# spaceandtimefdn/blitzar

Hardware: NVIDIA H100
Metric: MSM throughput (scalar*point terms/sec), ristretto255, n=2^20 per GPU (higher is better)
Workload: dtype u32 limbs (integer modular arithmetic)

## Files before the change

### blitzar_b200/build.py

```python
import os
import subprocess
import sys

ROOT = os.path.dirname(os.path.dirname(os.path.abspath(__file__)))
CSRC = os.path.join(ROOT, "blitzar_b200", "csrc")
LIBDIR = os.path.join(ROOT, "blitzar_b200", "lib")
LIB = os.path.join(LIBDIR, "libblitzar_b200.so")
NVCC = os.environ.get("NVCC", "/usr/local/cuda/bin/nvcc")
ARCH = ["-gencode", "arch=compute_90a,code=sm_90a"]
NVCC_FLAGS = ["-std=c++17", "-O3"] + ARCH + ["-lineinfo",
              "--expt-relaxed-constexpr", "-Xcompiler", "-fPIC"]
UNITS = ["api.cu", "curve_ed25519.cu", "curve_bls12381.cu", "curve_bn254.cu", "curve_grumpkin.cu"]


def _newer(target, sources):
    if not os.path.exists(target):
        return True
    t = os.path.getmtime(target)
    return any(os.path.getmtime(s) > t for s in sources)


def _headers():
    return [os.path.join(CSRC, f) for f in os.listdir(CSRC) if f.endswith((".cuh", ".h"))] + \
        [os.path.join(ROOT, "include", "blitzar_b200.h")]
# ... 1 lines not shown

def build_product(verbose=False):
    os.makedirs(LIBDIR, exist_ok=True)
    subprocess.check_call([sys.executable, os.path.join(CSRC, "gen_constants.py")])
    units = [u for u in UNITS if os.path.exists(os.path.join(CSRC, u))]
    objs, procs = [], []
    for u in units:
        src = os.path.join(CSRC, u)
        obj = os.path.join(LIBDIR, u.replace(".cu", ".o"))
        objs.append(obj)
        if _newer(obj, [src, os.path.abspath(__file__)] + _headers()):
            cmd = [NVCC] + NVCC_FLAGS + (["-Xptxas", "-v"] if verbose else []) + ["-c", src, "-o", obj]
            procs.append((u, subprocess.Popen(cmd, stdout=subprocess.PIPE, stderr=subprocess.STDOUT)))
    for u, p in procs:
        out, _ = p.communicate()
        if verbose or p.returncode:
            sys.stderr.write(out.decode())
        if p.returncode:
            raise RuntimeError(f"nvcc failed for {u}")
    if procs or not os.path.exists(LIB):
        subprocess.check_call([NVCC, "-shared"] + ARCH + ["-o", LIB] + objs +
                              ["-Xlinker", "--version-script=" + os.path.join(CSRC, "export.map")])
    return LIB


def build_emul():
    edir = os.path.join(ROOT, "tests", "emul")
    out = os.path.join(edir, "libb200_emul.so")
    objdir = os.path.join(edir, "obj")
    os.makedirs(objdir, exist_ok=True)
    prefix = os.path.join(edir, "emul_prefix.h")
    flags = ["g++", "-std=c++17", "-O1", "-DB200_EMULATE", "-fPIC", "-w", "-include", prefix]
    jobs, objs = [], []
    harness = ["emul.cpp", "ptable_emul.cpp", "offsets_emul.cpp", "partition_msm_emul.cpp"]
    for u in [x for x in UNITS if x.startswith("curve_")] + harness:
        src = os.path.join(edir if u in harness else CSRC, u)
        obj = os.path.join(objdir, u.rsplit(".", 1)[0] + ".o")
        objs.append(obj)
        if _newer(obj, [src, prefix] + _headers()):
            jobs.append((u, subprocess.Popen(flags + ["-x", "c++", "-c", src, "-o", obj],
                                             stdout=subprocess.PIPE, stderr=subprocess.STDOUT)))
    for u, p in jobs:
        o, _ = p.communicate()
        if p.returncode:
            sys.stderr.write(o.decode())
            raise RuntimeError(f"emulation build failed for {u}")
    if jobs or not os.path.exists(out):
        subprocess.check_call(["g++", "-shared", "-o", out] + objs)
    return out


def build_oracle_port():
    src = os.path.join(ROOT, "oracle", "msm_oracle.c")
    out = os.path.join(ROOT, "oracle", "libmsm_oracle.so")
    if os.path.exists(src) and _newer(out, [src]):
        subprocess.check_call(["gcc", "-O2", "-fPIC", "-shared", "-w", src, "-o", out])
    return out


def build_oracle_ref():
    ref = os.environ.get("BLITZAR_REFERENCE")
    if not ref or not os.path.isdir(os.path.join(ref, "sxt")):
        return None
    subprocess.check_call(["make", "-s", "-j8", "-C", os.path.join(ROOT, "oracle", "ref_build"),
                           "R=" + os.path.abspath(ref)], stdout=subprocess.DEVNULL)
    return os.path.join(ROOT, "oracle", "_ref", "libblitzar_ref_cpu.so")

# ... 11 lines not shown
```

### blitzar_b200/csrc/api.cu

```cuda
#include <algorithm>
#include <cctype>
#include <cstdint>
#include <cstdio>
#include <cstdlib>
#include <cstring>
#include <condition_variable>
#include <functional>
#include <mutex>
#include <thread>
#include <memory>
#include <string>
#include <vector>

#include "engine_api.cuh"

using namespace b200;

namespace {

struct State {
  bool initialized = false;
  int device = -1;
  cudaStream_t stream = nullptr;
  cudaStream_t copy_stream = nullptr;
  cudaStream_t tail_stream = nullptr;
  cudaEvent_t range_events[16] = {};
  cudaEvent_t alloc_event = nullptr;
  void* builtin = nullptr;
  uint64_t num_builtin = 0;
  unsigned builtin_window_bits = 0, builtin_windows = 0;
  MsmOptions opt;
};
State g_state;
EngineCtx ctx_of(const State& st) {
  EngineCtx c{st.stream, g_state.opt, st.builtin, st.num_builtin};
  c.builtin_window_bits = st.builtin_window_bits;
  c.builtin_windows = st.builtin_windows;
  static const bool tail_on = [] {
    const char* env = std::getenv("BLITZAR_B200_TAIL_STREAM");
    return env != nullptr && std::atoi(env) != 0;
  }();
  if (tail_on)
    c.tail = st.tail_stream;
  if (const char* env = std::getenv("BLITZAR_B200_GROUP_ENTRIES"))
    c.opt.max_group_entries = std::strtoull(env, nullptr, 10);
  if (const char* env = std::getenv("BLITZAR_B200_UNIFORM_ADD"))
    c.opt.uniform_add = (u32)std::atoi(env);
  if (const char* env = std::getenv("BLITZAR_B200_LANE_TAIL"))
    c.opt.lane_tail = (u32)std::atoi(env);
  if (const char* env = std::getenv("BLITZAR_B200_SCATTER_WM"))
    c.opt.scatter_window_major = (u32)std::atoi(env);
  if (const char* env = std::getenv("BLITZAR_B200_SORT"))
    c.opt.sort_path = (u32)std::atoi(env);
  if (const char* env = std::getenv("BLITZAR_B200_PAIR_LEVELS"))
    c.opt.pair_levels = std::atoi(env);
  if (const char* env = std::getenv("BLITZAR_B200_PAIR_BATCH"))
    c.opt.pair_batch = (u32)std::atoi(env);
  if (const char* env = std::getenv("BLITZAR_B200_TABLE_POLICY"))
    c.opt.table_policy = (u32)std::atoi(env);
  if (const char* env = std::getenv("BLITZAR_B200_PARTITION_POLICY"))
    c.partition_policy = (u32)std::atoi(env);
  return c;
}
EngineCtx ctx() { return ctx_of(g_state); }
std::mutex g_mutex;

void init_device_state(State& st) {
  B200_CUDA(cudaSetDevice(st.device));
  B200_CUDA(cudaStreamCreateWithFlags(&st.stream, cudaStreamNonBlocking));
  B200_CUDA(cudaStreamCreateWithFlags(&st.copy_stream, cudaStreamNonBlocking));
  int prio_low = 0, prio_high = 0;
  B200_CUDA(cudaDeviceGetStreamPriorityRange(&prio_low, &prio_high));
  B200_CUDA(cudaStreamCreateWithPriority(&st.tail_stream, cudaStreamNonBlocking, prio_high));
  for (auto& e : st.range_events)
    B200_CUDA(cudaEventCreateWithFlags(&e, cudaEventDisableTiming));
  B200_CUDA(cudaEventCreateWithFlags(&st.alloc_event, cudaEventDisableTiming));
  cudaMemPool_t pool;
  B200_CUDA(cudaDeviceGetDefaultMemPool(&pool, st.device));
  uint64_t threshold = UINT64_MAX;
  B200_CUDA(cudaMemPoolSetAttribute(pool, cudaMemPoolAttrReleaseThreshold, &threshold));
}

void ensure_device() {
  if (g_state.stream)
    return;
  int count = 0;
// ... 1318 lines not shown
```

### blitzar_b200/csrc/curve.cuh

```cuda
#pragma once
#include "field.cuh"

namespace b200 {

enum CurveId : unsigned { kRistretto255 = 0, kBls12381 = 1, kBn254 = 2, kGrumpkin = 3 };

struct SeqExec {
  static constexpr int kLanes = 1;
  template <class F>
  static B200_HD void mul4(typename F::E& o0, typename F::E& o1, typename F::E& o2,
                           typename F::E& o3, const typename F::E& a0, const typename F::E& b0,
                           const typename F::E& a1, const typename F::E& b1,
                           const typename F::E& a2, const typename F::E& b2,
                           const typename F::E& a3, const typename F::E& b3) {
    F::mul(o0, a0, b0);
    F::mul(o1, a1, b1);
    F::mul(o2, a2, b2);
    F::mul(o3, a3, b3);
  }
  template <class F>
  static B200_HD void mul2(typename F::E& o0, typename F::E& o1, const typename F::E& a0,
                           const typename F::E& b0, const typename F::E& a1,
                           const typename F::E& b1) {
    F::mul(o0, a0, b0);
// ... 148 lines not shown
    F::select(qt, g.T2d, nt, negate);
    F::sub(t0, a.Y, a.X);
    F::add(t1, a.Y, a.X);
    if (unit_z) {
      F::mul(A, t0, qm);
      F::mul(B, t1, qp);
      F::mul(C, a.T, qt);
      F::dbl(D, a.Z);
    } else {
      X::template mul4<F>(A, B, C, D, t0, qm, t1, qp, a.T, qt, a.Z, g.Z2);
    }
    F::sub(E, B, A);
    F::sub(Fv, D, C);
    F::add(G, D, C);
    F::add(H, B, A);
    Point o;
    X::template mul4<F>(o.X, o.Y, o.T, o.Z, E, Fv, G, H, E, H, Fv, G);
    r = o;
  }
  template <class X = SeqExec> static B200_HD void dbl(Point& r, const Point& a) {
    fe A, B, C, E, Fv, G, H, t0, t1;
    F::add(t0, a.X, a.Y);
    X::template mul4<F>(A, B, C, t1, a.X, a.X, a.Y, a.Y, a.Z, a.Z, t0, t0);
    F::dbl(C, C);
    F::add(H, A, B);
    F::sub(E, H, t1);
    F::sub(G, A, B);
    F::add(Fv, C, G);
    Point o;
    X::template mul4<F>(o.X, o.Y, o.T, o.Z, E, Fv, G, H, E, H, Fv, G);
    r = o;
  }

  static B200_HD void load_gen_abi(Gen& g, const void* src) {
    const u64* s = (const u64*)src;
    Point p;
    F::from_radix51(p.X, s);
    F::from_radix51(p.Y, s + 5);
    F::from_radix51(p.Z, s + 10);
    F::from_radix51(p.T, s + 15);
    point_to_gen(g, p);
  }
  static B200_HD void load_proj_abi(Gen& g, const void* src) { load_gen_abi(g, src); }
  static constexpr int kAbiCompactBytes = 120;
  static B200_HD void load_compact_abi(Gen& g, const void* src) {
    const u64* s = (const u64*)src;
    Point p;
    F::from_radix51(p.X, s);
    F::from_radix51(p.Y, s + 5);
    p.Z = F::one();
    F::from_radix51(p.T, s + 10);
    point_to_gen(g, p);
  }
  static B200_HD void store_compact_abi(void* dst, const Point& p, const fe& zi) {
    u64* d = (u64*)dst;
    fe x, y, t;
    F::mul(x, p.X, zi);
    F::mul(y, p.Y, zi);
    F::mul(t, x, y);
    F::to_radix51(d, x);
    F::to_radix51(d + 5, y);
    F::to_radix51(d + 10, t);
  }
  static B200_HD void store_proj_abi(void* dst, const Point& p) {
    u64* d = (u64*)dst;
    F::to_radix51(d, p.X);
    F::to_radix51(d + 5, p.Y);
    F::to_radix51(d + 10, p.Z);
    F::to_radix51(d + 15, p.T);
  }

  struct ScalarPow {
    static B200_HD void pow22523(fe& r, const fe& a) { F::pow22523(r, a); }
// ... 464 lines not shown
```

### blitzar_b200/csrc/engine.cuh

```cuda
#pragma once
#include <cstdint>
#include <vector>

#include "engine_api.cuh"
#include "msm.cuh"
#include "partition_msm.cuh"
#include "ptable.cuh"
#include "synth.cuh"

namespace b200 {

inline uint64_t check_descriptors(const sxt_sequence_descriptor* d, uint32_t num) {
  B200_REQUIRE(d != nullptr, "descriptors == nullptr");
  uint64_t longest = 0;
  for (uint32_t i = 0; i < num; ++i) {
    B200_REQUIRE(d[i].n == 0 || d[i].data != nullptr, "descriptor.n > 0 with data == nullptr");
    B200_REQUIRE(d[i].element_nbytes != 0 && d[i].element_nbytes <= 32,
                 "descriptor.element_nbytes must be in 1..32");
    if (d[i].is_signed)
      B200_REQUIRE(d[i].element_nbytes <= 16 &&
                       (d[i].element_nbytes & (d[i].element_nbytes - 1)) == 0,
                   "signed columns need a power-of-two element_nbytes <= 16");
    B200_REQUIRE(d[i].n < (1ull << 31), "column too long");
    longest = longest < d[i].n ? d[i].n : longest;
// ... 9 lines not shown
                          Point* out, u32 num_ranges = 1, RangeHook* hook = nullptr) {
    const uint64_t kMaxEntries = ctx.opt.max_group_entries;
    size_t b = 0;
    while (b < cols.size()) {
      size_t e = b;
      uint64_t entries = 0;
      while (e < cols.size()) {
        uint64_t est = (uint64_t)cols[e].n * (cols[e].bit_width / 10 + 1);
        if (e > b && entries + est > kMaxEntries)
          break;
        entries += est;
        ++e;
      }
      std::vector<ColumnDesc> group(cols.begin() + b, cols.begin() + e);
      const bool whole = b == 0 && e == cols.size();
      if (!whole && hook && b == 0) {
        hook->before_range(0, ~0ull);
        hook->before_accumulate();
      }
      msm_run<C>(ctx.s, gens, group, out + b, ctx.opt, whole ? num_ranges : 1,
                 whole ? hook : nullptr, ctx.tail);
      b = e;
    }
  }

  struct IngestHook : RangeHook {
    const EngineCtx* ctx;
    const unsigned char* raw;
    Gen* gens;
    uint64_t n, offset_generators;
    bool builtin;
    range_wait_fn wait;
    void* wait_user;
    bool pending = false;
    void before_range(u64 begin, u64 end) override {
      if (end > n)
        end = n;
      if (begin >= end)
        return;
      if (wait)
        wait(wait_user, begin, end);
      if (raw) {
        stream_t aux = aux_stream();
        stream_follow(aux, ctx->s);
        launch(IngestBody<C, false>{raw + begin * C::kAbiGenBytes, gens + begin}, end - begin, aux);
        pending = true;
      } else if (builtin) {
        launch_builtin(ctx->s, gens + begin, offset_generators + begin, end - begin);
      }
    }
    void before_accumulate() override {
      if (pending) {
        stream_follow(ctx->s, aux_stream());
        pending = false;
      }
    }
  };
  static void launch_builtin(stream_t s, Gen* gens, uint64_t first, uint64_t count) {
    if constexpr (C::kCurveId == kRistretto255)
      launch(BuiltinGeneratorBody{gens, first}, count, s);
    else
      die("generators == nullptr", __FILE__, __LINE__);
  }

  struct PiecesHook : RangeHook {
    const EngineCtx* ctx;
    const GenLayout* layout;
    const unsigned char* raw;
    bool packed;
    bool generate;
    Gen* gens;
    range_wait_fn wait;
    void* wait_user;
    bool pending = false;
    void before_range(u64 begin, u64 end) override {
      end = std::min<u64>(end, layout->max_n);
      if (begin >= end)
        return;
      if (wait)
        wait(wait_user, begin, end);
      if (!raw && !generate)
        return;
      const std::vector<GenLayout::Piece> pieces = layout->needed(begin, end);
      const size_t np = pieces.size();
      std::vector<u64> block(3 * np + 1, 0);
      for (size_t k = 0; k < np; ++k) {
        block[k + 1] = block[k] + pieces[k].count;
        block[np + 1 + k] = raw && packed ? pieces[k].pos : pieces[k].src;
        block[2 * np + 1 + k] = pieces[k].pos;
      }
      const stream_t on = raw ? aux_stream() : ctx->s;
      if (raw)
        stream_follow(on, ctx->s);
      const u64* staged = (const u64*)stage_to_device(on, block.data(), block.size() * sizeof(u64));
      const GenPieces p{staged, staged + np + 1, staged + 2 * np + 1, (u32)np};
      if (raw) {
        launch(IngestPiecesBody<C>{raw, gens, p}, block[np], on);
        pending = true;
      } else if constexpr (C::kCurveId == kRistretto255) {
        launch(BuiltinPiecesBody{gens, p}, block[np], on);
      }
      dev_free((void*)staged, on);
    }
    void before_accumulate() override {
      if (pending) {
        stream_follow(ctx->s, aux_stream());
        pending = false;
      }
    }
  };

  static std::vector<ColumnDesc> columns_of(const sxt_sequence_descriptor* d, uint32_t num) {
    std::vector<ColumnDesc> cols(num);
    for (uint32_t i = 0; i < num; ++i) {
      cols[i].base = d[i].data;
      cols[i].row_stride = d[i].element_nbytes;
      cols[i].bit_offset = 0;
      cols[i].bit_width = 8u * d[i].element_nbytes;
      cols[i].n = (u32)d[i].n;
      cols[i].is_signed = d[i].is_signed ? 1u : 0u;
      cols[i].first_window = cols[i].num_windows = 0;
      cols[i].table_n = 0;
    }
    return cols;
  }

  static void commit_columns(const EngineCtx& ctx, void* out_commitments, void* out_partials,
                             std::vector<ColumnDesc>& cols, const Gen* gens, bool builtin_table,
                             uint32_t num_ranges, RangeHook* hook) {
    stream_t s = ctx.s;
// ... 13 lines not shown
    }
    run_columns(rctx, gens, cols, pts, num_ranges ? num_ranges : 1, hook);
    hook->before_accumulate();
    if (out_commitments)
      launch_store_commit<C>(s, pts, (unsigned char*)out_commitments, num, ctx.opt.lane_tail != 0);
  }

  static void commit_device(const EngineCtx& ctx, void* out_commitments, void* out_partials,
                            uint32_t num, const sxt_sequence_descriptor* d,
                            const void* generators_dev, uint64_t offset_generators,
                            uint32_t num_ranges, range_wait_fn wait, void* wait_user) {
    stream_t s = ctx.s;
    uint64_t n = check_descriptors(d, num);
    DevBuf<Gen> gens(n ? n : 1, s);
    const Gen* gens_ptr = gens.p;
    IngestHook hook;
    hook.ctx = &ctx;
    hook.raw = (const unsigned char*)generators_dev;
    hook.gens = gens.p;
    hook.n = n;
    hook.offset_generators = offset_generators;
    hook.builtin = false;
    hook.wait = wait;
    hook.wait_user = wait_user;
    if (n && !generators_dev) {
      if (C::kCurveId != kRistretto255)
        die("generators == nullptr", __FILE__, __LINE__);
      if (offset_generators + n <= ctx.num_builtin)
        gens_ptr = (const Gen*)ctx.builtin + offset_generators;
      else
        hook.builtin = true;
    }
    std::vector<ColumnDesc> cols = columns_of(d, num);
    commit_columns(ctx, out_commitments, out_partials, cols, gens_ptr,
                   n && !generators_dev && !hook.builtin, num_ranges, &hook);
  }

  static void commit_device_offsets(const EngineCtx& ctx, void* out_commitments,
                                    void* out_partials, uint32_t num,
                                    const sxt_sequence_descriptor* d, const void* generators_dev,
                                    const uint64_t* offsets, bool packed, uint32_t num_ranges,
                                    range_wait_fn wait, void* wait_user) {
    check_descriptors(d, num);
    const GenLayout layout(d, num, offsets);
    if (layout.total && !generators_dev && C::kCurveId != kRistretto255)
      die("generators == nullptr", __FILE__, __LINE__);
    const bool builtin_table = layout.total && !generators_dev && layout.within(ctx.num_builtin);
    DevBuf<Gen> gens(builtin_table ? 1 : layout.total, ctx.s);
    PiecesHook hook;
    hook.ctx = &ctx;
    hook.layout = &layout;
    hook.raw = (const unsigned char*)generators_dev;
    hook.packed = packed;
    hook.generate = layout.total && !generators_dev && !builtin_table;
    hook.gens = gens.p;
    hook.wait = wait;
    hook.wait_user = wait_user;
    std::vector<ColumnDesc> cols = columns_of(d, num);
    for (uint32_t j = 0; j < num; ++j)
      cols[j].gen_base = builtin_table && d[j].n && offsets ? (u32)offsets[j] : layout.base[j];
    commit_columns(ctx, out_commitments, out_partials, cols,
                   builtin_table ? (const Gen*)ctx.builtin : gens.p, builtin_table, num_ranges,
                   &hook);
  }

  static void fixed_device(const EngineCtx& ctx, void* out_res, void* out_partials, const Handle* h,
                           int mode, unsigned element_num_bytes, const unsigned* bit_table,
                           const unsigned* lengths, unsigned num_outputs, unsigned n,
                           const uint8_t* scalars_dev) {
    stream_t s = ctx.s;
    std::vector<ColumnDesc> cols(num_outputs);
    uint64_t row_bits = 0;
    if (mode == 0) {
      B200_REQUIRE(element_num_bytes >= 1 && element_num_bytes <= 32, "element_num_bytes in 1..32");
      row_bits = 8ull * element_num_bytes * num_outputs;
    } else {
      for (unsigned j = 0; j < num_outputs; ++j) {
        B200_REQUIRE(bit_table[j] > 0 && bit_table[j] <= 256, "output bit width must be in 1..256");
        row_bits += bit_table[j];
      }
    }
    const uint64_t row_stride = (row_bits + 7) / 8;
    uint64_t bit_off = 0;
    for (unsigned j = 0; j < num_outputs; ++j) {
      unsigned width = mode == 0 ? 8u * element_num_bytes : bit_table[j];
      unsigned len = mode == 2 ? lengths[j] : n;
      B200_REQUIRE(len <= h->n, "more scalars than generators in the handle");
      cols[j].base = scalars_dev;
      cols[j].row_stride = row_stride;
      cols[j].bit_offset = (u32)bit_off;
      cols[j].bit_width = width;
      cols[j].n = len;
      cols[j].is_signed = 0;
      cols[j].first_window = cols[j].num_windows = 0;
// ... 160 lines not shown
```

### blitzar_b200/csrc/engine_api.cuh

```cuda
#pragma once
#include <algorithm>
#include <cmath>
#include <cstdint>
#include <vector>

#include "../../include/blitzar_b200.h"
#include "runtime.cuh"

namespace b200 {

struct MsmOptions {
  u32 window_bits = 0;
  u32 chunk1 = 0;
  u32 chunkn = 8;
  u32 reduce_g1 = 16;
  u32 reduce_gn = 4;
  u64 quad_threshold = 32768;
  u64 max_group_entries = 1ull << 30;
  u64 max_range_entries = 1ull << 31;
  int pair_levels = -1;
  u32 pair_batch = 0;
  int range_skew = 0;
  u32 uniform_add = 2;
  u32 gens_normalized = 0;
  u32 lane_tail = 1;
  u32 scatter_window_major = 0;
  u32 sort_path = 1;
  u32 table_policy = 0;
};

struct EngineCtx {
  stream_t s;
  MsmOptions opt;
  const void* builtin;
  uint64_t num_builtin;
  stream_t tail = stream_t();
  u32 builtin_window_bits = 0, builtin_windows = 0;
  u32 partition_policy = 0;
};

struct Handle {
  unsigned curve_id;
  unsigned n;
  void* gens;
  unsigned window_bits = 0, windows = 1;
  void* ptable = nullptr;
  unsigned ptable_w = 0;
  uint64_t ptable_groups = 0;
};

inline unsigned table_window_bits(uint64_t n, size_t gen_bytes, double budget_bytes) {
  if (n < 1024)
    return 0;
  unsigned best = 0;
  double best_cost = 1e300;
  for (unsigned c = 10; c <= 20; ++c) {
    const double W = 256 / c + 1;
// ... 150 lines not shown
```

### blitzar_b200/csrc/msm.cuh

```cuda
#pragma once
#include <algorithm>
#include <vector>

#include "batch_affine.cuh"
#include "curve.cuh"
#include "engine_api.cuh"
#include "lanefield.cuh"

namespace b200 {

struct ColumnDesc {
  const unsigned char* base;
  u64 row_stride;
  u32 bit_offset;
  u32 bit_width;
  u32 n;
  u32 is_signed;
  u32 first_window;
  u32 num_windows;
  u32 table_n;
  u32 gen_base;
};
B200_HD u32 bucket_windows(const ColumnDesc& col) { return col.table_n ? (col.num_windows ? 1u : 0u) : col.num_windows; }

// ... 488 lines not shown
                        u64 nkeys, u64* entries, u32* counts, u32* d_m) {
  const u32 shift = binned_sort_shift(nkeys);
  const u32 nmicro = (u32)((nkeys + (1ull << shift) - 1) >> shift);
  const u32 span_micro = std::max(1u, kBinSpan >> shift);
  u32* ws = (u32*)dev_alloc((5ull * nmicro + 3) * sizeof(u32), s);
  u32 *micro_counts = ws, *bin_of = ws + nmicro, *bin_cursor = ws + 2ull * nmicro,
      *bin_start = ws + 3ull * nmicro, *bin_micro = ws + 4ull * nmicro + 1,
      *nbins = ws + 5ull * nmicro + 2;
  u64* tmp = (u64*)dev_alloc(std::max<u64>(max_entries, 1) * sizeof(u64), s);
  dev_zero(micro_counts, nmicro * sizeof(u32), s);
  const u64 count_tile = 4096;
  launch_blocks(MicroCountBody{d_cols, d_col_start, ncols, c, nbuckets, total_terms,
                               (u32)count_tile, shift, nmicro, micro_counts},
                (total_terms + count_tile - 1) / count_tile, nmicro * sizeof(u32), s);
  launch_blocks(PlanBinsBody{micro_counts, nmicro, span_micro, nkeys, bin_of, bin_start, bin_micro,
                             bin_cursor, nbins, counts, d_m},
                1, nmicro * sizeof(u32), s);
  const size_t scatter_smem = 220 * 1024;
  const size_t bin_bytes = (2ull * nmicro + 2) * sizeof(u32);
  const u64 stage_entries = (scatter_smem - bin_bytes) / sizeof(u64);
  const u64 scatter_tile = std::max<u64>(1, stage_entries / max_windows);
  launch_blocks(CoarseScatterBody{d_cols, d_col_start, ncols, c, nbuckets, total_terms,
                                  (u32)scatter_tile, shift, nmicro, bin_of, nbins, bin_cursor, tmp},
                (total_terms + scatter_tile - 1) / scatter_tile, scatter_smem, s);
  launch_blocks(BinSortBody{tmp, bin_start, bin_micro, nbins, shift, nkeys, entries, counts}, nmicro,
                BinSortBody::kSmem, s);
  dev_free(tmp, s);
  dev_free(ws, s);
}
#endif

template <class C> struct FillIdentityBody {
  static constexpr int kBlock = 256;
  typename C::Point* p;
  B200_HD void operator()(u64 t) const { p[t] = C::identity(); }
};

template <class C> struct MergeBucketsBody {
  static constexpr int kBlock = 128;
  const u32* bucket_end;
  const u32* bucket_begin;
  const typename C::Point* scratch;
  typename C::Point* buckets;
  B200_HD void operator()(u64 k) const {
    const u32 lo = bucket_begin ? bucket_begin[k] : (k ? bucket_end[k - 1] : 0u);
    if (bucket_end[k] == lo)
      return;
    typename C::Point b = buckets[k];
    C::add(b, b, scratch[k]);
    buckets[k] = b;
  }
};

template <class C, bool kGather, class X = SeqExec, bool kUniform = false> struct AccumulateBody {
  static constexpr int kBlock = 128;
  static constexpr int kMinBlocks = !kGather ? 1 : (C::F::N > 8 ? 2 : 3);
  typedef typename C::Point Point;
  const u32* keys;
  const u64* entries;
  const typename C::Gen* gens;
  const Point* pieces;
  const u32* m_ptr;
  u32 K;
  u32 final_level;
  Point* buckets;
  u32* out_keys;
  Point* out_pieces;
  u32* out_m_ptr;
  u32 unit_z;

  B200_HD void put_bucket(u32 key, const Point& acc, bool writer) const {
    if (writer)
      buckets[key] = acc;
  }
  B200_HD u32 key_at(u64 i) const { return kGather ? (u32)(entries[i] >> 32) : keys[i]; }
  B200_HD void fetch(Point& acc, u64 i, bool first) const {
    if (kGather) {
      u32 e = (u32)entries[i];
      if (first)
        C::gen_to_point(acc, gens[e >> 1], e & 1u);
      else
        C::template add_gen<X>(acc, acc, gens[e >> 1], e & 1u);
    } else {
      if (first)
        acc = pieces[i];
      else
        C::template add<X>(acc, acc, pieces[i]);
    }
  }
  B200_HD void operator()(u64 tid) const {
    const u64 t = tid / X::kLanes;
    const bool writer = (tid % X::kLanes) == 0;
    const u64 M = *m_ptr;
    const u64 T = (M + K - 1) / K;
    if (tid == 0 && out_m_ptr)
      *out_m_ptr = final_level ? 0u : (u32)(2 * T);
    u64 b = t * K;
    if (b >= M)
      return;
    u64 e = b + K < M ? b + K : M;
    u32 cur;
    Point acc;
    bool first_seg = true;
    if (kGather) {
      u64 ent = entries[b];
      typename C::Gen g = gens[(u32)ent >> 1];
      cur = (u32)(ent >> 32);
      struct {
        Point p;
        bool unit;
        B200_HD void start(const typename C::Gen& g, bool negate) { C::gen_to_point(p, g, negate); }
        B200_HD void add(const typename C::Gen& g, bool negate) {
          C::template add_gen<X>(p, p, g, negate, unit);
        }
        B200_HD void get(Point& out) const { out = p; }
      } ga;
      ga.unit = unit_z != 0;
      for (u64 i = b; i < e; ++i) {
        u64 ent_n = ent;
        typename C::Gen g_n = g;
        if (i + 1 < e) {
          ent_n = entries[i + 1];
          g_n = gens[(u32)ent_n >> 1];
        }
        const u32 k = (u32)(ent >> 32);
        const bool negate = ((u32)ent & 1u) != 0;
        if (kUniform) {
          if (i == b) {
            ga.p = C::identity();
          } else if (k != cur) {
            ga.get(acc);
            if (final_level || !first_seg) {
              put_bucket(cur, acc, writer);
            } else if (writer) {
              out_keys[2 * t] = cur;
              out_pieces[2 * t] = acc;
            }
            first_seg = false;
            cur = k;
            ga.p = C::identity();
          }
          ga.add(g, negate);
        } else if (i == b) {
          ga.start(g, negate);
        } else if (k == cur) {
          ga.add(g, negate);
        } else {
          ga.get(acc);
          if (final_level || !first_seg) {
            put_bucket(cur, acc, writer);
          } else if (writer) {
            out_keys[2 * t] = cur;
            out_pieces[2 * t] = acc;
          }
          first_seg = false;
          cur = k;
          ga.start(g, negate);
        }
        ent = ent_n;
        g = g_n;
      }
      ga.get(acc);
    } else {
      cur = key_at(b);
      fetch(acc, b, true);
      for (u64 i = b + 1; i < e; ++i) {
        u32 k = key_at(i);
        if (k == cur) {
          fetch(acc, i, false);
        } else {
          if (final_level || !first_seg) {
            put_bucket(cur, acc, writer);
          } else if (writer) {
            out_keys[2 * t] = cur;
            out_pieces[2 * t] = acc;
          }
          first_seg = false;
          cur = k;
          fetch(acc, i, true);
        }
      }
    }
    if (final_level) {
      put_bucket(cur, acc, writer);
      return;
    }
    if (!writer)
      return;
    if (first_seg) {
      out_keys[2 * t] = cur;
      out_pieces[2 * t] = acc;
      out_keys[2 * t + 1] = cur;
      out_pieces[2 * t + 1] = C::identity();
    } else {
      out_keys[2 * t + 1] = cur;
// ... 229 lines not shown
  Ed25519::Gen* gens;
  u64 first;
  B200_HD void operator()(u64 i) const {
    Ed25519::Point g;
    Ed25519::builtin_generator(g, first + i);
    Ed25519::point_to_gen(gens[i], g);
  }
};
struct GenPieces {
  const u64* start;
  const u64* from;
  const u64* to;
  u32 npieces;
};
template <class C> struct IngestPiecesBody {
  static constexpr int kBlock = IngestBody<C, false>::kBlock;
  const unsigned char* raw;
  typename C::Gen* gens;
  GenPieces p;
  B200_HD void operator()(u64 tid) const {
    const u32 k = column_of(p.start, p.npieces, tid);
    IngestBody<C, false>{raw + p.from[k] * C::kAbiGenBytes, gens + p.to[k]}(tid - p.start[k]);
  }
};
struct BuiltinPiecesBody {
  static constexpr int kBlock = BuiltinGeneratorBody::kBlock;
  Ed25519::Gen* gens;
  GenPieces p;
  B200_HD void operator()(u64 tid) const {
    const u32 k = column_of(p.start, p.npieces, tid);
    BuiltinGeneratorBody{gens + p.to[k], p.from[k]}(tid - p.start[k]);
  }
};
template <class C, bool kCommit> struct StoreBody {
  static constexpr int kBlock = 32;
  const typename C::Point* pts;
  unsigned char* out;
  B200_HD void operator()(u64 i) const {
    if (kCommit)
      C::store_commit_abi(out + i * C::kAbiCommitBytes, pts[i]);
    else
      C::store_proj_abi(out + i * C::kAbiProjBytes, pts[i]);
  }
};
template <class C>
inline void launch_store_commit(stream_t s, const typename C::Point* pts, unsigned char* out,
                                u64 count, bool lane_tail) {
#ifdef B200_LANE_TAIL
  if constexpr (C::kCurveId == kRistretto255) {
    if (lane_tail && count && count <= 4096) {
      launch(StoreLaneBody{pts, out, count}, (count + 2) / 3 * 32, s);
      return;
    }
  }
#endif
  launch(StoreBody<C, true>{pts, out}, count, s);
}
template <class C> struct GenToProjBody {
  static constexpr int kBlock = 64;
  const typename C::Gen* gens;
  unsigned char* out;
  B200_HD void operator()(u64 i) const {
    typename C::Point p;
    C::gen_to_point(p, gens[i], false);
    C::store_proj_abi(out + i * C::kAbiProjBytes, p);
  }
// ... 166 lines not shown
  copy_d2h(ca.data(), a.counts, (nkeys + 1) * sizeof(u32), s);
  copy_d2h(cb.data(), b.counts, (nkeys + 1) * sizeof(u32), s);
  copy_d2h(m.data(), b.d_m, sizeof(u32), s);
  copy_d2h(ea.data(), a.entries, M * sizeof(u64), s);
  copy_d2h(eb.data(), b.entries, M * sizeof(u64), s);
  stream_sync(s);
  for (void* p : {(void*)a.entries, (void*)a.counts, (void*)a.d_m, (void*)b.entries, (void*)b.counts,
                  (void*)b.d_m, (void*)r.d_cols})
    dev_free(p, s);
  if (!b.binned)
    return ~0u;
  unsigned bad = m[0] == ca[nkeys] ? 0u : 1u;
  for (u64 k = 0; k < nkeys; ++k) {
    const u32 lo = k ? ca[k - 1] : 0u, hi = ca[k];
    if (cb[k] != hi || hi < lo || hi > M) {
      ++bad;
      continue;
    }
    std::sort(ea.begin() + lo, ea.begin() + hi);
    std::sort(eb.begin() + lo, eb.begin() + hi);
    if (!std::equal(ea.begin() + lo, ea.begin() + hi, eb.begin() + lo))
      ++bad;
  }
  return bad;
}

struct RangeHook {
  virtual void before_range(u64 begin, u64 end) = 0;
  virtual void before_accumulate() {}
  virtual ~RangeHook() {}
};

template <class C>
stream_t chunk_walk(stream_t s, stream_t tail, WalkInput<C> walk, u32* d_m, u32 unit_z,
                    typename C::Point* target, const MsmOptions& opt, std::vector<void*>& to_free) {
  typedef typename C::Point Point;
  u32 K = opt.chunk1 ? std::max(opt.chunk1, 4u) : (walk.m_max >= (1ull << 23) ? 64u : 32u);
  const u32 chunkn = std::max(opt.chunkn, 4u);
  const u32* lvl_keys = nullptr;
  const Point* lvl_pieces = nullptr;
  stream_t cs = s;
  for (int level = 0;; ++level) {
    const bool final_level = walk.m_max <= K;
    u64 T = (walk.m_max + K - 1) / K;
    u32* out_keys = final_level ? nullptr : (u32*)dev_alloc(2 * T * sizeof(u32), cs);
    Point* out_pieces = final_level ? nullptr : (Point*)dev_alloc(2 * T * sizeof(Point), cs);
    to_free.insert(to_free.end(), {out_keys, out_pieces});
    u32* out_m = d_m + 1 + (level % 8);
    if (level == 0) {
      const bool uniform =
          opt.uniform_add == 2 ? C::kCurveId == kRistretto255 : opt.uniform_add != 0;
      if (uniform)
        launch(AccumulateBody<C, true, SeqExec, true>{nullptr, walk.entries, walk.gens, nullptr,
                                                      walk.m_ptr, K, final_level, target, out_keys,
                                                      out_pieces, out_m, unit_z},
               T, s);
      else
        launch(AccumulateBody<C, true>{nullptr, walk.entries, walk.gens, nullptr, walk.m_ptr, K,
                                       final_level, target, out_keys, out_pieces, out_m, unit_z},
               T, s);
      KernelTimer::get().end(s);
      if (tail != s)
        stream_follow(tail, s);
      cs = tail;
    } else if (T <= opt.quad_threshold) {
      launch(AccumulateBody<C, false, QuadExec>{lvl_keys, nullptr, nullptr, lvl_pieces, walk.m_ptr,
                                                K, final_level, target, out_keys, out_pieces, out_m, 0u},
             T * QuadExec::kLanes, cs);
    } else {
      launch(AccumulateBody<C, false>{lvl_keys, nullptr, nullptr, lvl_pieces, walk.m_ptr, K,
                                      final_level, target, out_keys, out_pieces, out_m, 0u},
             T, cs);
    }
    if (final_level)
      break;
    lvl_keys = out_keys;
    lvl_pieces = out_pieces;
    walk.m_ptr = out_m;
    walk.m_max = 2 * T;
    K = chunkn;
  }
  return cs;
}

template <class C>
void msm_accumulate_range(stream_t s, const MsmPlan& plan, const typename C::Gen* gens, u64 begin,
                          u64 end, bool add_into, typename C::Point* d_buckets,
                          u32* d_window_used, const MsmOptions& opt, stream_t tail,
                          RangeHook* hook = nullptr) {
  const StagedRange r(s, plan, begin, end);
  if (r.total_terms == 0)
    return;
  gens += begin;
  StageRange nvtx_sort("msm: digit count + scan + scatter");
  const u64 max_entries = r.max_entries, nkeys = plan.nkeys;
  u32 L = 0;
  if constexpr (C::kBatchAffine) {
    const double mean = (double)max_entries / (double)nkeys;
    if (opt.pair_levels >= 0)
      L = (u32)opt.pair_levels;
    else if (max_entries >= (1ull << 23))
      while (L < 6 && (double)(32u << L) <= mean)
        ++L;
    while (L > 0 && max_entries + nkeys * ((1ull << L) - 1) >= (1ull << 32) - (1ull << L))
      --L;
  }
  const SortedLayout sorted = sort_entries(s, plan, r, L, opt, d_window_used);
  B200_LOG(3, "range [%llu, %llu): %llu terms, %llu entries max, c=%u, %llu keys, pair levels %u",
           (unsigned long long)begin, (unsigned long long)end, (unsigned long long)r.total_terms,
           (unsigned long long)max_entries, plan.c, (unsigned long long)nkeys, L);
  WalkInput<C> walk{gens, sorted.entries, sorted.d_m, max_entries};
  std::vector<void*> to_free;
  if (hook)
    hook->before_accumulate();
  KernelTimer::get().begin(s);
  StageRange nvtx_acc("msm: bucket accumulation");
  if constexpr (C::kBatchAffine) {
    if (L) {
      walk = run_pair_levels<C>(s, L, sorted.entries, gens, sorted.d_m, sorted.slots_max,
                                opt.pair_batch);
      to_free = {(void*)walk.gens, (void*)walk.entries};
    }
  }
  typedef typename C::Point Point;
  Point* target = add_into ? (Point*)dev_alloc(nkeys * sizeof(Point), s) : d_buckets;
  const u32 unit_z = (walk.gens == gens && opt.gens_normalized) ? 1u : 0u;
  const stream_t cs = chunk_walk<C>(s, tail, walk, sorted.d_m, unit_z, target, opt, to_free);
  if (add_into) {
    launch(MergeBucketsBody<C>{sorted.counts, sorted.starts, target, d_buckets}, nkeys, cs);
    dev_free(target, cs);
  }
  to_free.insert(to_free.end(), {sorted.d_m, sorted.counts, sorted.starts});
  for (void* ptr : to_free)
    dev_free(ptr, cs);
  dev_free(sorted.entries, s);
  dev_free((void*)r.d_cols, s);
}

template <class C>
void msm_finish(stream_t s, const MsmPlan& plan, const typename C::Point* d_buckets,
                const u32* d_window_used, typename C::Point* out, const MsmOptions& opt) {
  typedef typename C::Point Point;
  StageRange nvtx_fin("msm: bucket reduction + window combination");
  const u32 total_windows = plan.total_windows, nbuckets = plan.nbuckets, ncols = plan.ncols;
  ColumnDesc* d_cols =
      (ColumnDesc*)stage_to_device(s, plan.cols.data(), ncols * sizeof(ColumnDesc));
  Point* d_S = nullptr;
  u32 m = nbuckets;
  const Point* X = d_buckets;
  const Point* Cin = nullptr;
  std::vector<void*> to_free;
  if (m == 1) {
    d_S = (Point*)dev_alloc(total_windows * sizeof(Point), s);
    copy_d2d(d_S, d_buckets, total_windows * sizeof(Point), s);
  }
  bool first = true;
  while (m > 1) {
    u32 g = first ? std::min<u32>(opt.reduce_g1, m) : std::min<u32>(opt.reduce_gn, m);
    u32 log2g = 0;
    while ((1u << log2g) < g)
// ... 29 lines not shown
      launch(CombineLaneBody{d_S, d_cols, plan.c, out}, (u64)ncols * 32, s);
      lane_done = true;
    }
  }
  if (lane_done) {
  } else
#endif
  if (ncols <= opt.quad_threshold && uniform_windows)
    launch(CombineBody<C, QuadExecConv>{d_S, d_cols, plan.c, out}, (u64)ncols * QuadExec::kLanes,
           s);
  else if (ncols <= opt.quad_threshold)
    launch(CombineBody<C, QuadExec>{d_S, d_cols, plan.c, out}, (u64)ncols * QuadExec::kLanes, s);
  else
    launch(CombineBody<C>{d_S, d_cols, plan.c, out}, ncols, s);
  dev_free(d_S, s);
  dev_free(d_cols, s);
}

template <class C>
void msm_run(stream_t s, const typename C::Gen* gens, std::vector<ColumnDesc> cols,
             typename C::Point* out, const MsmOptions& opt = MsmOptions(), u32 num_ranges = 1,
             RangeHook* hook = nullptr, stream_t tail = stream_t()) {
  typedef typename C::Point Point;
  if (cols.empty())
    return;
  MsmPlan plan = msm_make_plan(std::move(cols), opt, sizeof(Point));
  B200_LOG(2, "msm: curve %u, %u columns, longest %llu, %llu terms, window %u bits, %u bucket sets%s",
           C::kCurveId, plan.ncols, (unsigned long long)plan.max_n,
           (unsigned long long)plan.total_terms, plan.c, plan.total_windows,
           plan.ncols && plan.cols[0].table_n ? " (fixed-base table)" : "");
  if (plan.total_terms == 0 || plan.total_windows == 0) {
    if (hook)
      hook->before_range(0, plan.max_n);
    launch(FillIdentityBody<C>{out}, plan.ncols, s);
    return;
  }
  Point* d_buckets = (Point*)dev_alloc(plan.nkeys * sizeof(Point), s);
  launch(FillIdentityBody<C>{d_buckets}, plan.nkeys, s);
  u32* d_window_used = (u32*)dev_alloc(plan.total_windows * sizeof(u32), s);
  dev_zero(d_window_used, plan.total_windows * sizeof(u32), s);
  if (num_ranges < 1)
    num_ranges = 1;
  const u64 limit = opt.max_range_entries ? opt.max_range_entries : (1ull << 31);
  const u64 needed = (plan.total_entries + limit - 1) / limit;
  if (needed > num_ranges)
    num_ranges = (u32)std::min<u64>(needed, plan.max_n);
  const bool overlap = num_ranges > 1 && tail != stream_t() && tail != s;
  for (u32 r = 0; r < num_ranges; ++r) {
    u64 begin = range_begin(plan.max_n, r, num_ranges, opt.range_skew),
        end = range_begin(plan.max_n, r + 1, num_ranges, opt.range_skew);
    if (hook)
      hook->before_range(begin, end);
    msm_accumulate_range<C>(s, plan, gens, begin, end, r > 0, d_buckets, d_window_used, opt,
                            overlap ? tail : s, hook);
  }
  if (overlap)
    stream_follow(s, tail);
  msm_finish<C>(s, plan, d_buckets, d_window_used, out, opt);
  dev_free(d_window_used, s);
  dev_free(d_buckets, s);
}

}
```

Baseline: 301.0 million.

## Normalize ristretto generators to Z=1 on ingest and use unit-Z mixed adds

Adds a batch-inversion pass at generator ingest that scales each ristretto255 generator to Z=1, so the bucket accumulation kernel can use a cheaper mixed addition with the Z term fixed at 2 instead of loading it. A device flag vetoes the unit path when any input Z is zero, and normalization is on by default. The identity fill is also rewritten to write 16-byte chunks per thread for coalescing. The trade is extra ingest work (prefix products plus one inversion) against fewer multiplications in each bucket add.

```diff
diff --git a/blitzar_b200/build.py b/blitzar_b200/build.py
--- a/blitzar_b200/build.py
+++ b/blitzar_b200/build.py
@@ -57,7 +57,8 @@
     prefix = os.path.join(edir, "emul_prefix.h")
     flags = ["g++", "-std=c++17", "-O1", "-DB200_EMULATE", "-fPIC", "-w", "-include", prefix]
     jobs, objs = [], []
-    harness = ["emul.cpp", "ptable_emul.cpp", "offsets_emul.cpp", "partition_msm_emul.cpp"]
+    harness = ["emul.cpp", "ptable_emul.cpp", "offsets_emul.cpp", "partition_msm_emul.cpp",
+               "normalize_emul.cpp"]
     for u in [x for x in UNITS if x.startswith("curve_")] + harness:
         src = os.path.join(edir if u in harness else CSRC, u)
         obj = os.path.join(objdir, u.rsplit(".", 1)[0] + ".o")
diff --git a/blitzar_b200/csrc/api.cu b/blitzar_b200/csrc/api.cu
--- a/blitzar_b200/csrc/api.cu
+++ b/blitzar_b200/csrc/api.cu
@@ -52,6 +52,8 @@
     c.opt.scatter_window_major = (u32)std::atoi(env);
   if (const char* env = std::getenv("BLITZAR_B200_SORT"))
     c.opt.sort_path = (u32)std::atoi(env);
+  if (const char* env = std::getenv("BLITZAR_B200_NORMALIZE_GENS"))
+    c.opt.normalize_gens = (u32)std::atoi(env);
   if (const char* env = std::getenv("BLITZAR_B200_PAIR_LEVELS"))
     c.opt.pair_levels = std::atoi(env);
   if (const char* env = std::getenv("BLITZAR_B200_PAIR_BATCH"))
diff --git a/blitzar_b200/csrc/curve.cuh b/blitzar_b200/csrc/curve.cuh
--- a/blitzar_b200/csrc/curve.cuh
+++ b/blitzar_b200/csrc/curve.cuh
@@ -204,13 +204,31 @@
     r = o;
   }
 
-  static B200_HD void load_gen_abi(Gen& g, const void* src) {
+  static B200_HD Gen load_unit_gen(const Gen* src) {
+    Gen g;
+    g.YpX = src->YpX;
+    g.YmX = src->YmX;
+    g.T2d = src->T2d;
+    g.Z2 = F::zero();
+    g.Z2.l[0] = 2;
+    return g;
+  }
+
+  static B200_HD void load_point_abi(Point& p, const void* src) {
     const u64* s = (const u64*)src;
-    Point p;
     F::from_radix51(p.X, s);
     F::from_radix51(p.Y, s + 5);
     F::from_radix51(p.Z, s + 10);
     F::from_radix51(p.T, s + 15);
+  }
+  static B200_HD fe load_abi_z(const void* src) {
+    fe z;
+    F::from_radix51(z, (const u64*)src + 10);
+    return z;
+  }
+  static B200_HD void load_gen_abi(Gen& g, const void* src) {
+    Point p;
+    load_point_abi(p, src);
     point_to_gen(g, p);
   }
   static B200_HD void load_proj_abi(Gen& g, const void* src) { load_gen_abi(g, src); }
diff --git a/blitzar_b200/csrc/engine.cuh b/blitzar_b200/csrc/engine.cuh
--- a/blitzar_b200/csrc/engine.cuh
+++ b/blitzar_b200/csrc/engine.cuh
@@ -65,6 +65,7 @@
     bool builtin;
     range_wait_fn wait;
     void* wait_user;
+    u32* invalid = nullptr;
     bool pending = false;
     void before_range(u64 begin, u64 end) override {
       if (end > n)
@@ -76,6 +77,14 @@
       if (raw) {
         stream_t aux = aux_stream();
         stream_follow(aux, ctx->s);
+        if constexpr (C::kCurveId == kRistretto255) {
+          if (invalid) {
+            ingest_normalized(aux, raw + begin * C::kAbiGenBytes, gens + begin, IngestMap{},
+                              end - begin, invalid);
+            pending = true;
+            return;
+          }
+        }
         launch(IngestBody<C, false>{raw + begin * C::kAbiGenBytes, gens + begin}, end - begin, aux);
         pending = true;
       } else if (builtin) {
@@ -105,6 +114,7 @@
     Gen* gens;
     range_wait_fn wait;
     void* wait_user;
+    u32* invalid = nullptr;
     bool pending = false;
     void before_range(u64 begin, u64 end) override {
       end = std::min<u64>(end, layout->max_n);
@@ -127,8 +137,16 @@
         stream_follow(on, ctx->s);
       const u64* staged = (const u64*)stage_to_device(on, block.data(), block.size() * sizeof(u64));
       const GenPieces p{staged, staged + np + 1, staged + 2 * np + 1, (u32)np};
+      bool normalized = false;
+      if constexpr (C::kCurveId == kRistretto255) {
+        if (raw && invalid) {
+          ingest_normalized(on, raw, gens, IngestMap{p}, block[np], invalid);
+          normalized = true;
+        }
+      }
       if (raw) {
-        launch(IngestPiecesBody<C>{raw, gens, p}, block[np], on);
+        if (!normalized)
+          launch(IngestPiecesBody<C>{raw, gens, p}, block[np], on);
         pending = true;
       } else if constexpr (C::kCurveId == kRistretto255) {
         launch(BuiltinPiecesBody{gens, p}, block[np], on);
@@ -208,9 +226,26 @@
         hook.builtin = true;
     }
     std::vector<ColumnDesc> cols = columns_of(d, num);
-    commit_columns(ctx, out_commitments, out_partials, cols, gens_ptr,
+    const Normalizing norm(ctx, n && generators_dev, &hook.invalid);
+    commit_columns(norm.ctx, out_commitments, out_partials, cols, gens_ptr,
                    n && !generators_dev && !hook.builtin, num_ranges, &hook);
   }
+  struct Normalizing {
+    EngineCtx ctx;
+    u32* flag = nullptr;
+    Normalizing(const EngineCtx& c, bool ingests, u32** hook_invalid) : ctx(c) {
+      if (C::kCurveId != kRistretto255 || !ingests || !c.opt.normalize_gens)
+        return;
+      flag = (u32*)dev_alloc(sizeof(u32), c.s);
+      dev_zero(flag, sizeof(u32), c.s);
+      *hook_invalid = flag;
+      ctx.opt.gens_normalized = 1u;
+      ctx.opt.unit_veto = flag;
+    }
+    ~Normalizing() { dev_free(flag, ctx.s); }
+    Normalizing(const Normalizing&) = delete;
+    Normalizing& operator=(const Normalizing&) = delete;
+  };
 
   static void commit_device_offsets(const EngineCtx& ctx, void* out_commitments,
                                     void* out_partials, uint32_t num,
@@ -235,7 +270,8 @@
     std::vector<ColumnDesc> cols = columns_of(d, num);
     for (uint32_t j = 0; j < num; ++j)
       cols[j].gen_base = builtin_table && d[j].n && offsets ? (u32)offsets[j] : layout.base[j];
-    commit_columns(ctx, out_commitments, out_partials, cols,
+    const Normalizing norm(ctx, layout.total && generators_dev, &hook.invalid);
+    commit_columns(norm.ctx, out_commitments, out_partials, cols,
                    builtin_table ? (const Gen*)ctx.builtin : gens.p, builtin_table, num_ranges,
                    &hook);
   }
diff --git a/blitzar_b200/csrc/engine_api.cuh b/blitzar_b200/csrc/engine_api.cuh
--- a/blitzar_b200/csrc/engine_api.cuh
+++ b/blitzar_b200/csrc/engine_api.cuh
@@ -23,6 +23,8 @@
   int range_skew = 0;
   u32 uniform_add = 2;
   u32 gens_normalized = 0;
+  const u32* unit_veto = nullptr;
+  u32 normalize_gens = 1;
   u32 lane_tail = 1;
   u32 scatter_window_major = 0;
   u32 sort_path = 1;
diff --git a/blitzar_b200/csrc/msm.cuh b/blitzar_b200/csrc/msm.cuh
--- a/blitzar_b200/csrc/msm.cuh
+++ b/blitzar_b200/csrc/msm.cuh
@@ -544,9 +544,23 @@
 
 template <class C> struct FillIdentityBody {
   static constexpr int kBlock = 256;
-  typename C::Point* p;
-  B200_HD void operator()(u64 t) const { p[t] = C::identity(); }
-};
+  static constexpr u32 kChunks = sizeof(typename C::Point) / 16;
+  static_assert(sizeof(typename C::Point) % 16 == 0, "points are made of 16-byte aligned fields");
+  uint4* p;
+  B200_HD void operator()(u64 t) const {
+    const typename C::Point id = C::identity();
+    const u32 k = (u32)(t % kChunks);
+    uint4 v = ((const uint4*)&id)[0];
+#pragma unroll
+    for (u32 j = 1; j < kChunks; ++j)
+      if (j == k)
+        v = ((const uint4*)&id)[j];
+    p[t] = v;
+  }
+};
+template <class C> inline void fill_identity(stream_t s, typename C::Point* p, u64 n) {
+  launch(FillIdentityBody<C>{(uint4*)p}, n * FillIdentityBody<C>::kChunks, s);
+}
 
 template <class C> struct MergeBucketsBody {
   static constexpr int kBlock = 128;
@@ -564,13 +578,15 @@
   }
 };
 
-template <class C, bool kGather, class X = SeqExec, bool kUniform = false> struct AccumulateBody {
+template <class C, bool kGather, class X = SeqExec, bool kUniform = false, bool kUnitZ = false>
+struct AccumulateBody {
   static constexpr int kBlock = 128;
   static constexpr int kMinBlocks = !kGather ? 1 : (C::F::N > 8 ? 2 : 3);
   typedef typename C::Point Point;
+  typedef typename C::Gen Gen;
   const u32* keys;
   const u64* entries;
-  const typename C::Gen* gens;
+  const Gen* gens;
   const Point* pieces;
   const u32* m_ptr;
   u32 K;
@@ -579,7 +595,7 @@
   u32* out_keys;
   Point* out_pieces;
   u32* out_m_ptr;
-  u32 unit_z;
+  const u32* unit_veto;
 
   B200_HD void put_bucket(u32 key, const Point& acc, bool writer) const {
     if (writer)
@@ -599,6 +615,72 @@
       else
         C::template add<X>(acc, acc, pieces[i]);
     }
+  }
+  template <bool kUnit> B200_HD Gen load_gen(u32 idx) const {
+    if constexpr (kUnit)
+      return C::load_unit_gen(gens + idx);
+    else
+      return gens[idx];
+  }
+  template <bool kUnit>
+  B200_HD void gather_walk(u64 t, u64 b, u64 e, bool writer, u32& cur, Point& acc,
+                           bool& first_seg) const {
+    u64 ent = entries[b];
+    Gen g = load_gen<kUnit>((u32)ent >> 1);
+    cur = (u32)(ent >> 32);
+    struct {
+      Point p;
+      B200_HD void start(const Gen& g, bool negate) { C::gen_to_point(p, g, negate); }
+      B200_HD void add(const Gen& g, bool negate) {
+        C::template add_gen<X>(p, p, g, negate, kUnit);
+      }
+      B200_HD void get(Point& out) const { out = p; }
+    } ga;
+    for (u64 i = b; i < e; ++i) {
+      u64 ent_n = ent;
+      Gen g_n = g;
+      if (i + 1 < e) {
+        ent_n = entries[i + 1];
+        g_n = load_gen<kUnit>((u32)ent_n >> 1);
+      }
+      const u32 k = (u32)(ent >> 32);
+      const bool negate = ((u32)ent & 1u) != 0;
+      if (kUniform) {
+        if (i == b) {
+          ga.p = C::identity();
+        } else if (k != cur) {
+          ga.get(acc);
+          if (final_level || !first_seg) {
+            put_bucket(cur, acc, writer);
+          } else if (writer) {
+            out_keys[2 * t] = cur;
+            out_pieces[2 * t] = acc;
+          }
+          first_seg = false;
+          cur = k;
+          ga.p = C::identity();
+        }
+        ga.add(g, negate);
+      } else if (i == b) {
+        ga.start(g, negate);
+      } else if (k == cur) {
+        ga.add(g, negate);
+      } else {
+        ga.get(acc);
+        if (final_level || !first_seg) {
+          put_bucket(cur, acc, writer);
+        } else if (writer) {
+          out_keys[2 * t] = cur;
+          out_pieces[2 * t] = acc;
+        }
+        first_seg = false;
+        cur = k;
+        ga.start(g, negate);
+      }
+      ent = ent_n;
+      g = g_n;
+    }
+    ga.get(acc);
   }
   B200_HD void operator()(u64 tid) const {
     const u64 t = tid / X::kLanes;
@@ -615,64 +697,10 @@
     Point acc;
     bool first_seg = true;
     if (kGather) {
-      u64 ent = entries[b];
-      typename C::Gen g = gens[(u32)ent >> 1];
-      cur = (u32)(ent >> 32);
-      struct {
-        Point p;
-        bool unit;
-        B200_HD void start(const typename C::Gen& g, bool negate) { C::gen_to_point(p, g, negate); }
-        B200_HD void add(const typename C::Gen& g, bool negate) {
-          C::template add_gen<X>(p, p, g, negate, unit);
-        }
-        B200_HD void get(Point& out) const { out = p; }
-      } ga;
-      ga.unit = unit_z != 0;
-      for (u64 i = b; i < e; ++i) {
-        u64 ent_n = ent;
-        typename C::Gen g_n = g;
-        if (i + 1 < e) {
-          ent_n = entries[i + 1];
-          g_n = gens[(u32)ent_n >> 1];
-        }
-        const u32 k = (u32)(ent >> 32);
-        const bool negate = ((u32)ent & 1u) != 0;
-        if (kUniform) {
-          if (i == b) {
-            ga.p = C::identity();
-          } else if (k != cur) {
-            ga.get(acc);
-            if (final_level || !first_seg) {
-              put_bucket(cur, acc, writer);
-            } else if (writer) {
-              out_keys[2 * t] = cur;
-              out_pieces[2 * t] = acc;
-            }
-            first_seg = false;
-            cur = k;
-            ga.p = C::identity();
-          }
-          ga.add(g, negate);
-        } else if (i == b) {
-          ga.start(g, negate);
-        } else if (k == cur) {
-          ga.add(g, negate);
-        } else {
-          ga.get(acc);
-          if (final_level || !first_seg) {
-            put_bucket(cur, acc, writer);
-          } else if (writer) {
-            out_keys[2 * t] = cur;
-            out_pieces[2 * t] = acc;
-          }
-          first_seg = false;
-          cur = k;
-          ga.start(g, negate);
-        }
-        ent = ent_n;
-        g = g_n;
-      }
-      ga.get(acc);
+      if (kUnitZ && unit_veto && *unit_veto)
+        gather_walk<false>(t, b, e, writer, cur, acc, first_seg);
+      else
+        gather_walk<kUnitZ>(t, b, e, writer, cur, acc, first_seg);
     } else {
       cur = key_at(b);
       fetch(acc, b, true);
@@ -968,6 +996,223 @@
     BuiltinGeneratorBody{gens + p.to[k], p.from[k]}(tid - p.start[k]);
   }
 };
+
+struct IngestMap {
+  GenPieces p;
+  B200_HD void at(u64 i, u64& src, u64& dst) const {
+    if (p.npieces == 0) {
+      src = dst = i;
+      return;
+    }
+    const u32 k = column_of(p.start, p.npieces, i);
+    src = p.from[k] + (i - p.start[k]);
+    dst = p.to[k] + (i - p.start[k]);
+  }
+};
+constexpr u32 kNormBlock = 256;
+struct NormalizeUpBody {
+  static constexpr int kBlock = 128;
+  typedef F25519 F;
+  const unsigned char* raw;
+  IngestMap map;
+  u64 n, T;
+  F::E* pre;
+  F::E* prod;
+  u32* invalid;
+  B200_HD F::E group(u64 j) const {
+    F::E z[kBatchGroup], acc = F::one();
+#pragma unroll
+    for (u32 k = 0; k < kBatchGroup; ++k) {
+      const u64 i = j + k * T;
+      z[k] = F::one();
+      if (i < n) {
+        u64 src, dst;
+        map.at(i, src, dst);
+        z[k] = Ed25519::load_abi_z(raw + src * Ed25519::kAbiGenBytes);
+      }
+    }
+#pragma unroll
+    for (u32 k = 0; k < kBatchGroup; ++k) {
+      const u64 i = j + k * T;
+      if (i >= n)
+        break;
+      if (F::is_zero(z[k])) {
+        *invalid = 1u;
+        z[k] = F::one();
+      }
+      pre[i] = acc;
+      F::mul(acc, acc, z[k]);
+    }
+    return acc;
+  }
+  B200_HD void operator()(u64 j) const { prod[j] = group(j); }
+};
+struct NormalizeDownBody {
+  static constexpr int kBlock = 128;
+  typedef F25519 F;
+  const unsigned char* raw;
+  IngestMap map;
+  u64 n, T;
+  const F::E* pre;
+  const F::E* prod;
+  const F::E* ps;
+  const u32* invalid;
+  Ed25519::Gen* gens;
+  B200_HD void operator()(u64 j) const {
+    const bool scale = *invalid == 0;
+    F::E inv = prod[ps ? j / kNormBlock : j];
+    if (ps)
+      F::mul(inv, inv, ps[j]);
+    for (u32 k = kBatchGroup; k-- > 0;) {
+      const u64 i = j + k * T;
+      if (i >= n)
+        continue;
+      u64 src, dst;
+      map.at(i, src, dst);
+      Ed25519::Point p;
+      Ed25519::load_point_abi(p, raw + src * Ed25519::kAbiGenBytes);
+      if (scale) {
+        F::E zi;
+        F::mul(zi, inv, pre[i]);
+        F::mul(inv, inv, p.Z);
+        F::mul(p.X, p.X, zi);
+        F::mul(p.Y, p.Y, zi);
+        F::mul(p.T, p.T, zi);
+        p.Z = F::one();
+      }
+      Ed25519::Gen g;
+      Ed25519::point_to_gen(g, p);
+      gens[dst] = g;
+    }
+  }
+};
+#ifdef B200_BINNED_SORT
+__device__ __forceinline__ F25519::E shfl_up_fe(const F25519::E& a, u32 d) {
+  F25519::E r;
+#pragma unroll
+  for (int k = 0; k < 8; ++k)
+    r.l[k] = __shfl_up_sync(0xffffffffu, a.l[k], d);
+  return r;
+}
+__device__ __forceinline__ F25519::E shfl_down_fe(const F25519::E& a, u32 d) {
+  F25519::E r;
+#pragma unroll
+  for (int k = 0; k < 8; ++k)
+    r.l[k] = __shfl_down_sync(0xffffffffu, a.l[k], d);
+  return r;
+}
+template <int kBlock>
+__device__ void block_prefix_suffix(const F25519::E& x, F25519::E& P, F25519::E& S,
+                                    F25519::E& total, F25519::E* ws) {
+  typedef F25519 F;
+  const u32 lane = threadIdx.x & 31u, warp = threadIdx.x >> 5;
+  F::E inc = x, sinc = x;
+#pragma unroll
+  for (u32 d = 1; d < 32; d <<= 1) {
+    const F::E y = shfl_up_fe(inc, d), z = shfl_down_fe(sinc, d);
+    if (lane >= d)
+      F::mul(inc, inc, y);
+    if (lane + d < 32)
+      F::mul(sinc, sinc, z);
+  }
+  F::E pe = shfl_up_fe(inc, 1), se = shfl_down_fe(sinc, 1);
+  if (lane == 0)
+    pe = F::one();
+  if (lane == 31) {
+    se = F::one();
+    ws[warp] = inc;
+  }
+  __syncthreads();
+  F::E before = F::one(), after = F::one();
+  for (u32 w = 0; w < kBlock / 32; ++w) {
+    if (w < warp)
+      F::mul(before, before, ws[w]);
+    else if (w > warp)
+      F::mul(after, after, ws[w]);
+  }
+  F::mul(P, before, pe);
+  F::mul(S, se, after);
+  F::mul(total, before, ws[warp]);
+  F::mul(total, total, after);
+  __syncthreads();
+}
+struct NormalizeUpBlockBody {
+  static constexpr int kBlock = kNormBlock;
+  typedef F25519 F;
+  NormalizeUpBody up;
+  F::E* ps;
+  F::E* prod;
+  __device__ void run(u32 b, unsigned char*) const {
+    __shared__ F::E ws[kBlock / 32];
+    const u64 j = (u64)b * kBlock + threadIdx.x;
+    const F::E g = j < up.T ? up.group(j) : F::one();
+    F::E P, S, total;
+    block_prefix_suffix<kBlock>(g, P, S, total, ws);
+    if (j < up.T)
+      F::mul(ps[j], P, S);
+    if (threadIdx.x == 0)
+      prod[b] = total;
+  }
+};
+struct NormalizeMidBody {
+  static constexpr int kBlock = 1024;
+  typedef F25519 F;
+  F::E* vals;
+  F::E* pre;
+  u64 m;
+  __device__ void run(u32, unsigned char*) const {
+    __shared__ F::E ws[kBlock / 32];
+    __shared__ F::E inv_total;
+    const u64 per = (m + kBlock - 1) / kBlock, lo = min((u64)threadIdx.x * per, m),
+              hi = min(lo + per, m);
+    F::E c = F::one();
+    for (u64 k = lo; k < hi; ++k) {
+      pre[k] = c;
+      F::mul(c, c, vals[k]);
+    }
+    F::E P, S, total;
+    block_prefix_suffix<kBlock>(c, P, S, total, ws);
+    if (threadIdx.x == 0)
+      F::invert(inv_total, total);
+    __syncthreads();
+    F::E inv;
+    F::mul(inv, inv_total, P);
+    F::mul(inv, inv, S);
+    for (u64 k = hi; k-- > lo;) {
+      const F::E v = vals[k];
+      F::mul(vals[k], inv, pre[k]);
+      F::mul(inv, inv, v);
+    }
+  }
+};
+#endif
+inline void ingest_normalized(stream_t s, const unsigned char* raw, Ed25519::Gen* gens,
+                              const IngestMap& map, u64 n, u32* invalid) {
+  typedef F25519::E fe;
+  if (n == 0)
+    return;
+  const u64 T = (n + kBatchGroup - 1) / kBatchGroup;
+  fe* pre = (fe*)dev_alloc(n * sizeof(fe), s);
+  const NormalizeUpBody up{raw, map, n, T, pre, nullptr, invalid};
+#ifdef B200_BINNED_SORT
+  const u64 blocks = (T + kNormBlock - 1) / kNormBlock;
+  fe* ps = (fe*)dev_alloc((T + 2 * blocks) * sizeof(fe), s);
+  fe* prod = ps + T;
+  launch_blocks(NormalizeUpBlockBody{up, ps, prod}, blocks, 0, s);
+  launch_blocks(NormalizeMidBody{prod, prod + blocks, blocks}, 1, 0, s);
+  launch(NormalizeDownBody{raw, map, n, T, pre, prod, ps, invalid, gens}, T, s);
+  dev_free(ps, s);
+#else
+  fe* prod = (fe*)dev_alloc(T * sizeof(fe), s);
+  NormalizeUpBody u = up;
+  u.prod = prod;
+  launch(u, T, s);
+  batch_invert<F25519>(s, prod, T);
+  launch(NormalizeDownBody{raw, map, n, T, pre, prod, nullptr, invalid, gens}, T, s);
+  dev_free(prod, s);
+#endif
+  dev_free(pre, s);
+}
 template <class C, bool kCommit> struct StoreBody {
   static constexpr int kBlock = 32;
   const typename C::Point* pts;
@@ -1200,8 +1445,9 @@
 };
 
 template <class C>
-stream_t chunk_walk(stream_t s, stream_t tail, WalkInput<C> walk, u32* d_m, u32 unit_z,
-                    typename C::Point* target, const MsmOptions& opt, std::vector<void*>& to_free) {
+stream_t chunk_walk(stream_t s, stream_t tail, WalkInput<C> walk, u32* d_m, bool unit,
+                    const u32* unit_veto, typename C::Point* target, const MsmOptions& opt,
+                    std::vector<void*>& to_free) {
   typedef typename C::Point Point;
   u32 K = opt.chunk1 ? std::max(opt.chunk1, 4u) : (walk.m_max >= (1ull << 23) ? 64u : 32u);
   const u32 chunkn = std::max(opt.chunkn, 4u);
@@ -1218,14 +1464,26 @@
     if (level == 0) {
       const bool uniform =
           opt.uniform_add == 2 ? C::kCurveId == kRistretto255 : opt.uniform_add != 0;
-      if (uniform)
+      constexpr bool kEd = C::kCurveId == kRistretto255;
+      const bool unit_path = kEd && unit;
+      if (uniform && unit_path)
+        launch(AccumulateBody<C, true, SeqExec, true, kEd>{nullptr, walk.entries, walk.gens, nullptr,
+                                                            walk.m_ptr, K, final_level, target,
+                                                            out_keys, out_pieces, out_m, unit_veto},
+               T, s);
+      else if (uniform)
         launch(AccumulateBody<C, true, SeqExec, true>{nullptr, walk.entries, walk.gens, nullptr,
                                                       walk.m_ptr, K, final_level, target, out_keys,
-                                                      out_pieces, out_m, unit_z},
+                                                      out_pieces, out_m, nullptr},
+               T, s);
+      else if (unit_path)
+        launch(AccumulateBody<C, true, SeqExec, false, kEd>{nullptr, walk.entries, walk.gens, nullptr,
+                                                             walk.m_ptr, K, final_level, target,
+                                                             out_keys, out_pieces, out_m, unit_veto},
                T, s);
       else
         launch(AccumulateBody<C, true>{nullptr, walk.entries, walk.gens, nullptr, walk.m_ptr, K,
-                                       final_level, target, out_keys, out_pieces, out_m, unit_z},
+                                       final_level, target, out_keys, out_pieces, out_m, nullptr},
                T, s);
       KernelTimer::get().end(s);
       if (tail != s)
@@ -1233,11 +1491,12 @@
       cs = tail;
     } else if (T <= opt.quad_threshold) {
       launch(AccumulateBody<C, false, QuadExec>{lvl_keys, nullptr, nullptr, lvl_pieces, walk.m_ptr,
-                                                K, final_level, target, out_keys, out_pieces, out_m, 0u},
+                                                K, final_level, target, out_keys, out_pieces, out_m,
+                                                nullptr},
              T * QuadExec::kLanes, cs);
     } else {
       launch(AccumulateBody<C, false>{lvl_keys, nullptr, nullptr, lvl_pieces, walk.m_ptr, K,
-                                      final_level, target, out_keys, out_pieces, out_m, 0u},
+                                      final_level, target, out_keys, out_pieces, out_m, nullptr},
              T, cs);
     }
     if (final_level)
@@ -1292,8 +1551,9 @@
   }
   typedef typename C::Point Point;
   Point* target = add_into ? (Point*)dev_alloc(nkeys * sizeof(Point), s) : d_buckets;
-  const u32 unit_z = (walk.gens == gens && opt.gens_normalized) ? 1u : 0u;
-  const stream_t cs = chunk_walk<C>(s, tail, walk, sorted.d_m, unit_z, target, opt, to_free);
+  const bool unit = walk.gens == gens && opt.gens_normalized;
+  const stream_t cs =
+      chunk_walk<C>(s, tail, walk, sorted.d_m, unit, opt.unit_veto, target, opt, to_free);
   if (add_into) {
     launch(MergeBucketsBody<C>{sorted.counts, sorted.starts, target, d_buckets}, nkeys, cs);
     dev_free(target, cs);
@@ -1389,11 +1649,11 @@
   if (plan.total_terms == 0 || plan.total_windows == 0) {
     if (hook)
       hook->before_range(0, plan.max_n);
-    launch(FillIdentityBody<C>{out}, plan.ncols, s);
+    fill_identity<C>(s, out, plan.ncols);
     return;
   }
   Point* d_buckets = (Point*)dev_alloc(plan.nkeys * sizeof(Point), s);
-  launch(FillIdentityBody<C>{d_buckets}, plan.nkeys, s);
+  fill_identity<C>(s, d_buckets, plan.nkeys);
   u32* d_window_used = (u32*)dev_alloc(plan.total_windows * sizeof(u32), s);
   dev_zero(d_window_used, plan.total_windows * sizeof(u32), s);
   if (num_ranges < 1)
```

Measured after the change: 321.6 million (median of 6 runs). +6.8%, better.
